# nv-tlabs/LION

Hardware: NVIDIA H100
Metric: shapes/sec (1000-step DDPM, 2048 latent pts, B=32) (higher is better)
Workload: dtype tf32 (fp32 storage/accumulate)

## Files before the change

include/lion_b200.h:

```cpp
#ifndef LION_B200_H
#define LION_B200_H
#include <stddef.h>
#ifdef __cplusplus
extern "C" {
#endif

typedef struct LionCtx LionCtx;
typedef struct LionModel LionModel;

int lion_version(void);
const char* lion_last_error(void);
int lion_ctx_create(int device, LionCtx** out);
int lion_ctx_destroy(LionCtx* ctx);
int lion_ctx_last_launches(LionCtx* ctx);
int lion_ctx_last_conv_group(LionCtx* ctx);
unsigned lion_ctx_generation(LionCtx* ctx);
int lion_ctx_timeline(LionCtx* ctx, unsigned long long* t_ns, char* names, int max_entries);
size_t lion_ctx_arena_bytes(LionCtx* ctx);
size_t lion_workspace_bytes(LionCtx* ctx);

int lion_avg_voxelize(const float* features, const int* coords, float* out, int* ind, int* cnt,
                      int B, int C, int N, int r, void* stream);
int lion_trilinear_devoxelize(const float* grid, const float* coords, float* out, int* inds, float* wgts,
                              int B, int C, int N, int r, int is_training, void* stream);
int lion_furthest_point_sampling(const float* coords, int* idx, int B, int N, int M, void* stream);
int lion_gather(const float* features, const int* idx, float* out, int B, int C, int N, int M, void* stream);
int lion_ball_query(const float* centers, const float* points, int* out, int B, int N, int M, float radius, int K,
                    void* stream);
int lion_grouping(const float* features, const int* idx, float* out, int B, int C, int N, int M, int U, void* stream);
int lion_three_nn_interpolate(const float* points, const float* centers, const float* centers_features, float* out,
                              int* idx, float* wgt, int B, int C, int N, int M, void* stream);
int lion_voxel_coords(const float* coords, float* norm_coords, int* vox, int B, int N, int r, int normalize, float eps,
                      void* stream);

int lion_avg_voxelize_backward(const float* grad_y , const int* ind , const int* cnt ,
                               float* grad_x , int B, int C, int N, int r, void* stream);
int lion_trilinear_devoxelize_backward(const float* grad_y , const int* inds , const float* wgts ,
                                       float* grad_x , int B, int C, int N, int r, void* stream);
int lion_grouping_backward(const float* grad_y , const int* idx , float* grad_x , int B, int C,
                           int N, int M, int U, void* stream);
int lion_three_nn_interpolate_backward(const float* grad_y , const int* idx , const float* wgt ,
                                       float* grad_x , int B, int C, int N, int M, void* stream);
int lion_gather_backward(const float* grad_y , const int* idx , float* grad_x , int B, int C, int N,
                         int M, void* stream);

enum { LION_KIND_UNET = 1, LION_KIND_PVCONV = 2, LION_KIND_SA = 3, LION_KIND_FP = 4, LION_KIND_ATTN = 5,
       LION_KIND_SHARED_MLP = 6, LION_KIND_GLOBAL_PRIOR = 7, LION_KIND_ADAGN = 8, LION_KIND_CONV3D = 9,
       LION_KIND_STYLE_ENC = 10 };
int lion_model_create(LionCtx* ctx, int kind, const int* desc, int ndesc, const float* const* params, int nparams,
                      LionModel** out);
int lion_model_destroy(LionModel* m);
int lion_model_refresh(LionModel* m);

int lion_unet_forward(LionModel* m, const float* x, const float* t, const float* style, const float* clip, float* out,
                      int B, int N, void* stream);
int lion_unet_cache_style(LionModel* m, const float* style, const float* clip, int B, void* stream);
int lion_style_encoder_forward(LionModel* m, const float* x, float* out, int B, int N, void* stream);
int lion_pvconv_fwd(LionModel* m, const float* features, const float* coords, const float* style, float* out,
                    int B, int N, void* stream);
int lion_sa_module_fwd(LionModel* m, const float* features, const float* coords, const float* style,
                       float* out_features, float* out_coords, int B, int N, void* stream);
int lion_fp_module_fwd(LionModel* m, const float* points_coords, const float* centers_coords,
                       const float* centers_features, const float* points_features, const float* style, float* out,
                       int B, int N, int M, void* stream);
int lion_linear_attention_fwd(LionModel* m, const float* x, float* out, int B, int N, void* stream);
int lion_shared_mlp_fwd(LionModel* m, const float* x, const float* style, float* out, int B, int R, void* stream);
int lion_adagn_fwd(LionModel* m, const float* x, const float* style, float* out, int B, int R, void* stream);
int lion_se3d_fwd(LionCtx* ctx, const float* w1, const float* w2, const float* x, float* out, int B, int C, int V, void* stream);
// ... 59 lines not shown
```

lion_b200/_lib.py:

```python
import ctypes as C
import os
import threading

import torch

_HERE = os.path.dirname(os.path.abspath(__file__))
LIB_PATH = os.path.join(_HERE, "csrc", "liblion_b200.so")


class LionError(RuntimeError):
    pass


_lib = None
_lock = threading.Lock()
c_f = C.c_void_p


def _proto(lib):
    i, f, sz, vp = C.c_int, C.c_float, C.c_size_t, C.c_void_p
    P = lambda *a: list(a)
    sig = {
        "lion_version": ([], i),
        "lion_last_error": ([], C.c_char_p),
        "lion_ctx_create": (P(i, C.POINTER(vp)), i),
        "lion_ctx_destroy": (P(vp), i),
        "lion_ctx_last_launches": (P(vp), i),
        "lion_ctx_last_conv_group": (P(vp), i),
        "lion_ctx_arena_bytes": (P(vp), sz),
        "lion_ctx_generation": (P(vp), C.c_uint),
        "lion_ctx_timeline": (P(vp, vp, vp, i), i),
        "lion_avg_voxelize": (P(vp, vp, vp, vp, vp, i, i, i, i, vp), i),
        "lion_trilinear_devoxelize": (P(vp, vp, vp, vp, vp, i, i, i, i, i, vp), i),
        "lion_furthest_point_sampling": (P(vp, vp, i, i, i, vp), i),
        "lion_gather": (P(vp, vp, vp, i, i, i, i, vp), i),
        "lion_ball_query": (P(vp, vp, vp, i, i, i, f, i, vp), i),
        "lion_grouping": (P(vp, vp, vp, i, i, i, i, i, vp), i),
        "lion_three_nn_interpolate": (P(vp, vp, vp, vp, vp, vp, i, i, i, i, vp), i),
        "lion_voxel_coords": (P(vp, vp, vp, i, i, i, i, f, vp), i),
        "lion_avg_voxelize_backward": (P(vp, vp, vp, vp, i, i, i, i, vp), i),
        "lion_trilinear_devoxelize_backward": (P(vp, vp, vp, vp, i, i, i, i, vp), i),
        "lion_grouping_backward": (P(vp, vp, vp, i, i, i, i, i, vp), i),
        "lion_three_nn_interpolate_backward": (P(vp, vp, vp, vp, i, i, i, i, vp), i),
        "lion_gather_backward": (P(vp, vp, vp, i, i, i, i, vp), i),
        "lion_model_create": (P(vp, i, C.POINTER(i), i, C.POINTER(vp), i, C.POINTER(vp)), i),
        "lion_model_destroy": (P(vp), i),
        "lion_model_refresh": (P(vp), i),
        "lion_unet_forward": (P(vp, vp, vp, vp, vp, vp, i, i, vp), i),
        "lion_unet_cache_style": (P(vp, vp, vp, i, vp), i),
        "lion_style_encoder_forward": (P(vp, vp, vp, i, i, vp), i),
        "lion_pvconv_fwd": (P(vp, vp, vp, vp, vp, i, i, vp), i),
        "lion_sa_module_fwd": (P(vp, vp, vp, vp, vp, vp, i, i, vp), i),
        "lion_fp_module_fwd": (P(vp, vp, vp, vp, vp, vp, vp, i, i, i, vp), i),
        "lion_linear_attention_fwd": (P(vp, vp, vp, i, i, vp), i),
        "lion_shared_mlp_fwd": (P(vp, vp, vp, vp, i, i, vp), i),
        "lion_global_prior_forward": (P(vp, vp, vp, vp, vp, i, vp), i),
        "lion_adagn_fwd": (P(vp, vp, vp, vp, i, i, vp), i),
        "lion_se3d_fwd": (P(vp, vp, vp, vp, vp, i, i, i, vp), i),
        "lion_swish_fwd": (P(vp, vp, sz, vp), i),
        "lion_ddpm_update": (P(vp, vp, vp, vp, vp, vp, f, sz, vp, i, vp), i),
        "lion_ddpm_set_step": (P(vp, vp, i, i, vp), i),
        "lion_ddpm_next_step": (P(vp, vp, i, vp), i),
        "lion_ddpm_fetch_noise": (P(vp, vp, vp, sz, vp), i),
        "lion_conv3d_gn_fwd": (P(vp, vp, vp, vp, vp, i, vp), i),
        "lion_pvconv_conv1_probe": (P(vp, vp, vp, i, vp, vp, vp, C.POINTER(i), i, i, vp), i),
        "lion_sa_mlp_probe": (P(vp, vp, vp, vp, i, vp, vp, vp, vp, vp, vp, C.POINTER(i), i, i, vp), i),
        "lion_pvconv_probe": (P(vp, vp, vp, vp, vp, vp, vp, vp, vp, vp, vp, vp, C.POINTER(i), i, i, vp), i),
        "lion_attention_probe": (P(vp, vp, vp, vp, vp, i, i, vp), i),
        "lion_global_prior_step": (P(vp, vp, vp, vp, vp, i, vp), i),
        "lion_workspace_bytes": (P(vp), sz),
        "lion_ddim_update": (P(vp, vp, vp, vp, vp, vp, sz, vp, vp), i),
        "lion_ddim_set_step": (P(vp, vp, vp, i, i, i, vp), i),
        "lion_ddim_next_step": (P(vp, vp, vp, i, i, vp), i),
        "lion_scheduler_step": (P(vp, vp, vp, vp, vp, vp, sz, vp), i),
        "lion_chamfer_forward": (P(vp, vp, vp, vp, vp, vp, i, i, i, vp), i),
        "lion_chamfer_pairwise": (P(vp, vp, vp, i, i, i, i, vp), i),
        "lion_chamfer_backward": (P(vp, vp, vp, vp, vp, vp, vp, vp, i, i, i, vp), i),
        "lion_emd_approx": (P(vp, vp, vp, i, i, i, vp), i),
        "lion_emd_approx_saved": (P(vp, vp, vp, vp, i, i, i, vp), i),
        "lion_emd_backward": (P(vp, vp, vp, vp, vp, vp, i, i, i, vp), i),
        "lion_emd_pairwise": (P(vp, vp, vp, i, i, i, i, vp), i),
# ... 162 lines not shown
```

lion_b200/csrc/common.cuh:

```cuda
#pragma once
#include <cuda_runtime.h>
#include <cstdint>
#include <cstdio>
#include <cstdarg>
#include <cstring>
#include <string>
#include <vector>
#include <mutex>

namespace lion {

enum : int { LION_OK = 0, LION_ERR_CUDA = -1, LION_ERR_ARG = -2, LION_ERR_OOM = -3, LION_ERR_STATE = -4 };

void set_error(const char* fmt, ...);
const char* get_error();

#define LION_CHECK_CUDA(expr)                                                          \
  do {                                                                                 \
    cudaError_t _e = (expr);                                                           \
    if (_e != cudaSuccess) {                                                           \
      lion::set_error("%s:%d: %s -> %s", __FILE__, __LINE__, #expr, cudaGetErrorString(_e)); \
      return lion::LION_ERR_CUDA;                                                      \
    }                                                                                  \
  } while (0)

#define LION_REQUIRE(cond, ...)                                                        \
  do {                                                                                 \
    if (!(cond)) {                                                                     \
      lion::set_error(__VA_ARGS__);                                                    \
      return lion::LION_ERR_ARG;                                                       \
    }                                                                                  \
  } while (0)

#define LION_TRY(expr)                                                                 \
  do {                                                                                 \
    int _r = (expr);                                                                   \
    if (_r != 0) return _r;                                                            \
  } while (0)

constexpr int LION_MAX_STAMPS = 256;
struct Ctx {
  int device = 0;
  int num_sms = 132;
  int l2_bytes = 50 << 20;
  cudaStream_t stream = nullptr;
  cudaStream_t aux = nullptr;
  char* base = nullptr;
  char* zgrid = nullptr;
  size_t zgrid_cap = 0, zgrid_need = 0;
  size_t cap = 0;
  size_t off = 0;
  size_t peak = 0;
  unsigned generation = 0;
  std::mutex* mu = nullptr;
  bool dry = false;
  int launches = 0;
  int conv_smem_cap = 0;
  int conv_group_blocks = 0;
  unsigned long long* d_stamps = nullptr;
  int n_stamps = 0;
  char stamp_names[LION_MAX_STAMPS][24];

  void reset() { off = 0; peak = 0; launches = 0; zgrid_need = 0; n_stamps = 0; }
  void* alloc(size_t bytes) {
    size_t a = (off + 255) & ~size_t(255);
    off = a + bytes;
    if (off > peak) peak = off;
    if (dry) return (void*)(uintptr_t)(0x1000 + a);
    return base + a;
  }
  template <typename T> T* alloc_n(size_t n) { return (T*)alloc(n * sizeof(T)); }
  size_t mark() const { return off; }
  void release(size_t m) { off = m; }
};

int ctx_reserve(Ctx* c, size_t bytes);

#define LION_LAUNCH_ON(ctx, stream, kernel, grid, block, smem, ...)                    \
  do {                                                                                 \
    if (!(ctx)->dry) {                                                                 \
      kernel<<<(grid), (block), (smem), (stream)>>>(__VA_ARGS__);                      \
      (ctx)->launches++;                                                               \
    }                                                                                  \
  } while (0)
#define LION_LAUNCH(ctx, kernel, grid, block, smem, ...) LION_LAUNCH_ON(ctx, (ctx)->stream, kernel, grid, block, smem, __VA_ARGS__)

static __global__ void k_stamp(unsigned long long* p) {
  unsigned long long t;
  asm volatile("mov.u64 %0, %%globaltimer;" : "=l"(t));
  *p = t;
}
inline void stamp(Ctx* c, cudaStream_t s, const char* name, int idx = -1) {
  if (!c->d_stamps || c->dry || c->n_stamps >= LION_MAX_STAMPS) return;
  const char* pre = s == c->aux ? "aux:" : "";
  if (idx >= 0) snprintf(c->stamp_names[c->n_stamps], 24, "%s%s%d", pre, name, idx);
  else snprintf(c->stamp_names[c->n_stamps], 24, "%s%s", pre, name);
  k_stamp<<<1, 1, 0, s>>>(c->d_stamps + c->n_stamps);
  c->n_stamps++;
}

inline int memset_async(Ctx* c, void* p, int v, size_t bytes, cudaStream_t s) {
  if (c->dry || bytes == 0) return 0;
  LION_CHECK_CUDA(cudaMemsetAsync(p, v, bytes, s));
  return 0;
}
inline int memset_async(Ctx* c, void* p, int v, size_t bytes) { return memset_async(c, p, v, bytes, c->stream); }
inline int memcpy_d2d(Ctx* c, void* d, const void* s, size_t bytes) {
  if (c->dry || bytes == 0) return 0;
  LION_CHECK_CUDA(cudaMemcpyAsync(d, s, bytes, cudaMemcpyDeviceToDevice, c->stream));
  return 0;
}
// ... 62 lines not shown
```

lion_b200/csrc/conv_tc.cu:

```cuda
#include <algorithm>

#include "common.cuh"
#include "model.cuh"
#include "wgmma.cuh"

namespace lion {
namespace tc {

using namespace sm90;

constexpr int CONSUMER_WARPS = 8;
constexpr int THREADS = 32 * CONSUMER_WARPS + 32;
__host__ __device__ constexpr int conv_threads(int BPW) { return BPW == 2 ? 32 * CONSUMER_WARPS + 128 : THREADS; }
constexpr int PRODUCER_REGS = 96, CONSUMER_REGS = 200;
constexpr int MAX_A_STAGES = 16;
constexpr int MAX_B_STAGES = 4;
constexpr int OCC_SMEM = 1024;
__host__ __device__ constexpr int tiles_per_item(int NT) { return NT <= 32 ? 4 : (NT <= 64 ? 2 : 1); }
constexpr int SMEM_BIAS = 128 * 4, SMEM_BARS = 64 * 8 + 128;
__host__ __device__ constexpr int smem_stat(int NT) { return CONSUMER_WARPS * 2 * NT * 4; }
__host__ __device__ constexpr int smem_pool(int NT, int TPG) { return TPG == 1 ? CONSUMER_WARPS * 2 * NT * 4 : 0; }
__host__ __device__ constexpr int smem_fixed(int NT, int TPG) {
  return SMEM_BIAS + smem_stat(NT) + smem_pool(NT, TPG) + SMEM_BARS + OCC_SMEM;
}

struct Params {
  const float4* in; const float* w; const float* bias; float4* out; double* ssum; double* ssq;
  int Gin, Gout_store, cout_pad;
  int rows;
  int p_begin, p_end;
  int ntile;
  int ntg, tpg;
  int tg_off[3];
  int tap_off[9];
  int r, rp, nzb, npl, nblk, ib;
  int halo;
  int KG, nchunk;
  int NT;
  int G;
  int B;
  int a_stage_bytes, b_stage_bytes, stage_rows;
  int a_stages;
  int b_stages;
  const unsigned char* occ;
  int occ_stride;
  float* pool_mm;
  int sched;
};

__host__ __device__ __forceinline__ int block_row(int k, int rp, int nzb, int npl) {
  const int x = k / npl, rem = k - x * npl, yb = rem / nzb, zb = rem - yb * nzb;
  return ((x + 1) * rp + 1 + 8 * yb) * rp + 1 + 8 * zb;
}

template <int KG, int TPG, int NT, int NB = 1>
__device__ __forceinline__ void issue_stage(float (*d)[NT / 2], const uint32_t* a_addr, uint32_t b_addr, uint32_t a_pitch,
                                            uint32_t a_sbo, const int* tap_off) {
  const uint64_t b0 = make_desc(b_addr, NT * 16, 128);
  uint64_t a0[NB];
#pragma unroll
  for (int k = 0; k < NB; ++k) a0[k] = make_desc(a_addr[k], a_pitch, a_sbo);
#pragma unroll
  for (int t = 0; t < TPG; ++t) {
    const uint64_t toff = (uint64_t)(int64_t)(TPG == 1 ? 0 : tap_off[t]);
#pragma unroll
    for (int ks = 0; ks < KG / 2; ++ks)
#pragma unroll
      for (int k = 0; k < NB; ++k)
        wgmma_tf32<NT>(d[k], a0[k] + toff + (uint64_t)((ks * 2 * a_pitch) >> 4), b0 + (uint64_t)(((t * KG + ks * 2) * NT * 16) >> 4), 1);
  }
}


struct Items {
  long long u, u_end; int ntile_total, B, G;
  int mode, m, q, n_p, n_q, c_i, i, big, k;
  __device__ __forceinline__ bool next(int& nt, long long& v0, int& ntile) {
    const long long per_nt = (long long)B * ntile_total;
    if (mode) {
      while (u >= u_end) {
        if (k >= m) return false;
        const int a0 = q * k / m, a1 = q * (k + 1) / m, b0 = (q + 1) * k / m, b1 = (q + 1) * (k + 1) / m;
        u = (long long)n_q * a0 + (long long)n_p * b0 + (long long)(i - c_i) * (a1 - a0) + (long long)c_i * (b1 - b0);
        u_end = u + (big ? b1 - b0 : a1 - a0);
        ++k;
      }
      nt = (int)(u / per_nt);
      v0 = u - (long long)nt * per_nt;
      const long long lim = (long long)(nt + 1) * per_nt;
      const long long e = u_end < lim ? u_end : lim;
      ntile = (int)(e - u);
      u = e;
      return true;
    }
    if (u >= u_end) return false;
    nt = (int)(u / per_nt);
// ... 1 lines not shown
    long long run = per_nt - v0;
    if (u_end - u < run) run = u_end - u;
    const long long k2 = (run + G - 1) / G;
    ntile = (int)((run + k2 - 1) / k2);
    u += ntile;
    return true;
  }
};
__device__ __forceinline__ Items make_items(long long U, int ntile_total, int B, int G, int sched) {
  const long long u_begin = U * blockIdx.x / gridDim.x, u_end = U * (blockIdx.x + 1) / gridDim.x;
  Items it{u_begin, u_end, ntile_total, B, G, 0, 0, 0, 0, 0, 0, 0, 0, 0};
  if (sched) {
    const int grid = (int)gridDim.x, q = (int)(U / grid), n_p = (int)(U - (long long)q * grid);
    const int tmax = q + (n_p ? 1 : 0);
    it.mode = 1; it.u = 0; it.u_end = 0;
    it.m = (tmax + G - 1) / G; it.q = q; it.n_p = n_p; it.n_q = grid - n_p;
    it.i = (int)blockIdx.x; it.c_i = (int)(u_begin - (long long)q * blockIdx.x);
    it.big = (int)(u_end - u_begin) > q; it.k = 0;
  }
  return it;
}

__device__ __forceinline__ void halo_mask(int p_lo, int rp, bool& ok_lo, bool& ok_hi) {
  const int p_hi = p_lo + 8;
  const int z0 = p_lo % rp, y0 = (p_lo / rp) % rp, z1 = p_hi % rp, y1 = (p_hi / rp) % rp;
  ok_lo = ok_lo && z0 >= 1 && z0 <= rp - 2 && y0 >= 1 && y0 <= rp - 2;
  ok_hi = ok_hi && z1 >= 1 && z1 <= rp - 2 && y1 >= 1 && y1 <= rp - 2;
}
template <int NT>
__device__ __forceinline__ void stat_add(float* s_stat, int cw, int lane, int col, float x0, float x1, float x2, float x3) {
  const float s0 = red8<0>(x0 + x2), s1 = red8<0>(x1 + x3);
  const float q0 = red8<0>(fmaf(x0, x0, x2 * x2)), q1 = red8<0>(fmaf(x1, x1, x3 * x3));
  if (lane < 4) {
    float* st = s_stat + (cw * 2) * NT + col;
    st[0] += s0; st[1] += s1; st[NT] += q0; st[NT + 1] += q1;
  }
}
template <int NT>
__device__ __forceinline__ void stat_flush(const Params& P, float* s_stat, int et, int b, int n0) {
  asm volatile("bar.sync 1, 256;" ::: "memory");
  if (et < NT) {
    float s = 0.f, qq = 0.f;
#pragma unroll
    for (int w = 0; w < CONSUMER_WARPS; ++w) {
      s += s_stat[(w * 2 + 0) * NT + et]; qq += s_stat[(w * 2 + 1) * NT + et];
      s_stat[(w * 2 + 0) * NT + et] = 0.0f; s_stat[(w * 2 + 1) * NT + et] = 0.0f;
    }
    atomicAdd(P.ssum + (size_t)b * P.cout_pad + n0 + et, (double)s);
    atomicAdd(P.ssq + (size_t)b * P.cout_pad + n0 + et, (double)qq);
  }
  asm volatile("bar.sync 1, 256;" ::: "memory");
}

template <int KG, int TPG, int NT, bool BLK, int BPW = 1>
__global__ void __launch_bounds__(conv_threads(BPW), 1) k_conv_tc(Params P) {
  constexpr int GT = BLK ? BPW : tiles_per_item(NT);
  constexpr int NTHR = conv_threads(BPW);
  constexpr bool SETREG = NTHR > THREADS;
  constexpr int NACC = NT / 2;
  extern __shared__ __align__(128) uint8_t smem[];
  uint8_t* sA = smem;
  const int A_STAGES = P.a_stages;
  uint8_t* sB = sA + (size_t)A_STAGES * P.a_stage_bytes;
  const int B_STAGES = P.b_stages;
  float* s_bias = (float*)(sB + (size_t)B_STAGES * P.b_stage_bytes);
  float* s_stat = s_bias + 128;
  float* s_pool = s_stat + CONSUMER_WARPS * 2 * NT;
  uint64_t* bars = (uint64_t*)((uint8_t*)s_stat + smem_stat(NT) + smem_pool(NT, TPG));
  volatile uint32_t* s_skip = (volatile uint32_t*)(bars + 64);
  uint8_t* s_occ = (uint8_t*)(bars + 64) + 128;
  const int tid = threadIdx.x, warp = tid >> 5, lane = tid & 31;

  const uint32_t bar_full_a = smem_u32(bars), bar_empty_a = smem_u32(bars + MAX_A_STAGES);
  const uint32_t bar_full_b = smem_u32(bars + 2 * MAX_A_STAGES), bar_empty_b = smem_u32(bars + 2 * MAX_A_STAGES + MAX_B_STAGES);

  if (P.Gin % KG != 0)
    for (int i = tid; i < A_STAGES * P.a_stage_bytes / 16; i += NTHR) ((float4*)sA)[i] = make_float4(0.f, 0.f, 0.f, 0.f);
  for (int i = tid; i < CONSUMER_WARPS * 2 * NT; i += NTHR) s_stat[i] = 0.0f;
  if (tid == 0) {
    for (int i = 0; i < A_STAGES; ++i) { mbar_init(bar_full_a + 8 * i, 1); mbar_init(bar_empty_a + 8 * i, CONSUMER_WARPS); }
    for (int i = 0; i < B_STAGES; ++i) { mbar_init(bar_full_b + 8 * i, 1); mbar_init(bar_empty_b + 8 * i, CONSUMER_WARPS); }
    asm volatile("fence.mbarrier_init.release.cluster;" ::: "memory");
  }
  asm volatile("fence.proxy.async.shared::cta;" ::: "memory");
  __syncthreads();

  const int ntile_total = P.ntile;
  const int n_nt = P.cout_pad / P.NT;
  const long long U = (long long)n_nt * P.B * ntile_total;
  const Items items0 = make_items(U, ntile_total, P.B, P.G, P.sched);

  if (warp >= CONSUMER_WARPS) {
    if constexpr (SETREG) {
      regs_dec<PRODUCER_REGS>();
      if (warp > CONSUMER_WARPS) return;
    }
    uint32_t sa = 0, pa = 0, sb = 0, pb = 0;
    const uint32_t bytes = (uint32_t)P.stage_rows * 16u;
    const uint32_t sA_addr = smem_u32(sA), sB_addr = smem_u32(sB);
    Items items = items0;
    int nt, ntile;
    long long v0;
    int occ_shape = -1;
    while (items.next(nt, v0, ntile)) {
      const float* wsrc = P.w + (size_t)nt * P.nchunk * P.ntg * (P.b_stage_bytes / 4);
      int my_b = 0, my_t = 0;
      if (lane < ntile) { const int vl = (int)v0 + lane; my_b = vl / ntile_total; my_t = vl - my_b * ntile_total; }
      for (int cc = 0; cc < P.nchunk; ++cc) {
        const int kg_real = min(KG, P.Gin - cc * KG);
        const size_t grp_lane = (size_t)(cc * KG + (lane < kg_real ? lane : 0));
        for (int tg = 0; tg < P.ntg; ++tg) {
          const bool may_skip = P.occ && !(cc == P.nchunk - 1 && tg == P.ntg - 1);
          mbar_wait<SETREG>(bar_empty_b + 8 * sb, pb ^ 1);
          if (lane == 0) {
            mbar_expect_tx(bar_full_b + 8 * sb, P.b_stage_bytes);
            bulk_g2s(sB_addr + sb * (uint32_t)P.b_stage_bytes, wsrc + (size_t)(cc * P.ntg + tg) * (P.b_stage_bytes / 4),
                     P.b_stage_bytes, bar_full_b + 8 * sb);
          }
          if (++sb == B_STAGES) { sb = 0; pb ^= 1; }
          for (int j = 0; j < ntile; ++j) {
            const int bj = __shfl_sync(0xffffffffu, my_b, j), tj = __shfl_sync(0xffffffffu, my_t, j);
            long long row0;
            uint32_t cnt = (uint32_t)P.stage_rows;
            if (!BLK) {
              row0 = (long long)P.p_begin + (long long)tj * 128 - P.halo + P.tg_off[tg];
            } else {
              row0 = (long long)block_row(tj * P.ib, P.rp, P.nzb, P.npl) - P.rp - 1 + P.tg_off[tg];
              if (row0 + cnt > (long long)P.rows) cnt = (uint32_t)(P.rows - row0);
            }
            const float4* in_lane = P.in + ((size_t)bj * P.Gin + grp_lane) * P.rows;
            mbar_wait<SETREG>(bar_empty_a + 8 * sa, pa ^ 1);
            bool empty = false;
            if (may_skip) {
              const unsigned char* occ_b = P.occ + (size_t)bj * P.occ_stride;
              if (P.occ_stride <= OCC_SMEM) {
                if (occ_shape != bj) {
                  __syncwarp();
                  for (int k = lane; k < P.occ_stride; k += 32) s_occ[k] = __ldg(occ_b + k);
                  __syncwarp();
                  occ_shape = bj;
                }
                occ_b = s_occ;
              }
              long long lo = row0 < 0 ? 0 : row0, hi = row0 + cnt - 1;
              if (hi > P.rows - 1) hi = P.rows - 1;
              unsigned any = 0;
              for (int k = (int)(lo >> 6); k <= (int)(hi >> 6); ++k) any |= occ_b[k];
              empty = (any == 0);
            }
            const uint32_t full = bar_full_a + 8 * sa;
            if (lane == 0) {
              s_skip[sa] = empty ? 1u : 0u;
              if (empty) asm volatile("mbarrier.arrive.release.cta.shared::cta.b64 _, [%0];" ::"r"(full) : "memory");
              else mbar_expect_tx(full, cnt * 16u * kg_real);
            }
            __syncwarp();
            if (!empty && lane < kg_real)
              bulk_g2s(sA_addr + sa * (uint32_t)P.a_stage_bytes + lane * bytes, in_lane + row0, cnt * 16u, full);
            if (++sa == (uint32_t)A_STAGES) { sa = 0; pa ^= 1; }
          }
        }
      }
    }
  } else {
    if constexpr (SETREG) regs_inc<CONSUMER_REGS>();
    const int cw = warp, wg = cw >> 2, wq = cw & 3;
    const int et = tid;
    const uint32_t a_pitch = (uint32_t)P.stage_rows * 16u;
    const uint32_t a_sbo = BLK ? (uint32_t)P.rp * 16u : 128u;
    const uint32_t a_ring = smem_u32(sA) + (BLK ? 0u : (uint32_t)(P.halo + 64 * wg) * 16u);
    const uint32_t b_ring = smem_u32(sB);
    const int r_lo = 64 * wg + 16 * wq + (lane >> 2);
    const int c_lo = 2 * (lane & 3);
    const bool odd = (lane & 1) != 0;
    float acc[GT][NACC];
    uint32_t sa = 0, pa = 0, sb = 0, pb = 0;
    Items items = items0;
    int nt, ntile;
    long long v0;
    auto release = [&](int& s, uint32_t bar0) {
      if (s >= 0) { if (lane == 0) mbar_arrive(bar0 + 8 * s); s = -1; }
    };
    while (items.next(nt, v0, ntile)) {
#pragma unroll
      for (int j = 0; j < GT; ++j)
#pragma unroll
        for (int i = 0; i < NACC; ++i) acc[j][i] = 0.0f;
      int g_f = 0, nbw = 0;
      uint32_t boff[GT];
      if (BLK) {
        const int g_b = (int)(v0 / ntile_total);
        g_f = (int)(v0 - (long long)g_b * ntile_total) * P.ib;
        const int nb = min(P.ib, P.nblk - g_f);
        nbw = (nb - wg + 1) / 2;
        const int s_f = block_row(g_f, P.rp, P.nzb, P.npl);
#pragma unroll
        for (int j = 0; j < GT; ++j) {
          const int k = 2 * j + wg < nb ? g_f + 2 * j + wg : g_f;
          boff[j] = (uint32_t)(block_row(k, P.rp, P.nzb, P.npl) - s_f + P.rp + 1) * 16u;
        }
      }
      int pend_a = -1, pend_b = -1;
      for (int cc = 0; cc < P.nchunk; ++cc) {
        for (int tg = 0; tg < P.ntg; ++tg) {
          mbar_wait<SETREG>(bar_full_b + 8 * sb, pb);
          const uint32_t b_addr = b_ring + sb * (uint32_t)P.b_stage_bytes;
#pragma unroll
          for (int j = 0; j < (BLK ? 1 : GT); ++j) {
            if (j < ntile) {
              mbar_wait<SETREG>(bar_full_a + 8 * sa, pa);
              const uint32_t a_addr = a_ring + sa * (uint32_t)P.a_stage_bytes;
              if (!s_skip[sa]) {
                wg_fence();
                if (!BLK) {
                  issue_stage<KG, TPG, NT>(&acc[j], &a_addr, b_addr, a_pitch, a_sbo, P.tap_off);
                } else {
                  uint32_t a_blk[GT];
#pragma unroll
                  for (int k = 0; k < GT; ++k) a_blk[k] = a_addr + boff[k];
                  issue_stage<KG, TPG, NT, GT>(acc, a_blk, b_addr, a_pitch, a_sbo, P.tap_off);
                }
                wg_commit();
                wg_wait<1>();
                release(pend_a, bar_empty_a);
                release(pend_b, bar_empty_b);
                pend_a = (int)sa;
              } else {
                int s = (int)sa;
                release(s, bar_empty_a);
              }
              if (++sa == (uint32_t)A_STAGES) { sa = 0; pa ^= 1; }
            }
          }
          if (pend_b >= 0) {
            wg_wait<0>();
            release(pend_a, bar_empty_a);
            release(pend_b, bar_empty_b);
          }
          if (pend_a >= 0) pend_b = (int)sb;
          else { int s = (int)sb; release(s, bar_empty_b); }
          if (++sb == B_STAGES) { sb = 0; pb ^= 1; }
        }
      }
      wg_wait<0>();
      release(pend_a, bar_empty_a);
      release(pend_b, bar_empty_b);
#pragma unroll
      for (int j = 0; j < GT; ++j) fence_regs<NACC>(acc[j]);

      const int n0 = nt * NT;
      asm volatile("bar.sync 1, 256;" ::: "memory");
      if (et < NT) s_bias[et] = P.bias ? P.bias[n0 + et] : 0.0f;
      asm volatile("bar.sync 1, 256;" ::: "memory");
      int b = (int)(v0 / ntile_total);
#pragma unroll
      for (int j = 0; j < GT; ++j) {
        if (j < (BLK ? nbw : ntile)) {
          int tj = 0, p_lo, p_hi;
          bool ok_lo, ok_hi;
          bool in_lo, in_hi;
          if (!BLK) {
            const long long vj = v0 + j;
            const int bj = (int)(vj / ntile_total);
            tj = (int)(vj - (long long)bj * ntile_total);
            if (bj != b) { if (P.ssum) stat_flush<NT>(P, s_stat, et, b, n0); b = bj; }
            p_lo = P.p_begin + tj * 128 + r_lo; p_hi = p_lo + 8;
            in_lo = p_lo < P.p_end; in_hi = p_hi < P.p_end;
            ok_lo = in_lo; ok_hi = in_hi;
            if (TPG != 1) halo_mask(p_lo, P.rp, ok_lo, ok_hi);
          } else {
            const int k = g_f + 2 * j + wg, x = k / P.npl, rem = k - x * P.npl, yb = rem / P.nzb, zb = rem - yb * P.nzb;
            const int y = 1 + 8 * yb + 2 * wq, z = 1 + 8 * zb + (lane >> 2);
            p_lo = ((x + 1) * P.rp + y) * P.rp + z; p_hi = p_lo + P.rp;
            ok_lo = y <= P.r && z <= P.r; ok_hi = y + 1 <= P.r && z <= P.r;
            in_lo = ok_lo; in_hi = ok_hi;
          }
#pragma unroll
          for (int i = 0; i < NT / 8; ++i) {
            const int col = 8 * i + c_lo;
            const float x0 = ok_lo ? acc[j][4 * i + 0] + s_bias[col] : 0.0f, x1 = ok_lo ? acc[j][4 * i + 1] + s_bias[col + 1] : 0.0f;
            const float x2 = ok_hi ? acc[j][4 * i + 2] + s_bias[col] : 0.0f, x3 = ok_hi ? acc[j][4 * i + 3] + s_bias[col + 1] : 0.0f;
            if (P.ssum) stat_add<NT>(s_stat, cw, lane, col, x0, x1, x2, x3);
            if (TPG == 1 && P.pool_mm) {
              const float mn0 = red8<1>(fminf(x0, x2)), mn1 = red8<1>(fminf(x1, x3));
              const float mx0 = red8<2>(fmaxf(x0, x2)), mx1 = red8<2>(fmaxf(x1, x3));
              if (lane < 4) {
                float* sp = s_pool + (cw * 2) * NT + col;
                sp[0] = mn0; sp[1] = mn1; sp[NT] = mx0; sp[NT + 1] = mx1;
              }
            } else {
              const float y0 = __shfl_xor_sync(0xffffffffu, odd ? x0 : x2, 1);
              const float y1 = __shfl_xor_sync(0xffffffffu, odd ? x1 : x3, 1);
              const int g = (n0 + 8 * i + (lane & 2) * 2) >> 2;
              if (g < P.Gout_store) {
// ... 84 lines not shown
  int cc = r % nchunk; r /= nchunk;
  int nt = (int)r;
  int tap = tg * tpg + t;
  int ci = (cc * KG + kg) * 4 + jj;
  float v = 0.0f;
  if (ci < cin_pad) v = wt[((size_t)tap * cin_pad + ci) * cout_pad + nt * NT + n];
  uint32_t u;
  asm("cvt.rna.tf32.f32 %0, %1;" : "=r"(u) : "f"(v));
  w[i] = __uint_as_float(u);
}

}

int conv_tc_prepare(Model* m, ConvW& w) {
  w.tc = ConvTcW();
  if (!(w.ntaps == 27 || w.ntaps == 1)) return 0;
  if (w.cout_pad < 32 || w.cout_pad % 32) return 0;
  ConvTcW t;
  t.NT = w.cout_pad < 128 ? w.cout_pad : 128;
  if (w.cout_pad % t.NT) return 0;
  t.ntg = w.ntaps == 27 ? 3 : 1;
  t.tpg = w.ntaps == 27 ? 9 : 1;
  const int G = w.cin_pad / 4;
  t.KG = (w.ntaps == 27 && t.NT > 64) ? 4 : 8;
  if (G < t.KG) t.KG = (G <= 2) ? 2 : ((G <= 4) ? 4 : 8);
  t.nchunk = (G + t.KG - 1) / t.KG;
  const size_t total = (size_t)(w.cout_pad / t.NT) * t.nchunk * t.ntg * t.tpg * t.KG * t.NT * 4;
  LION_TRY(m->dmalloc(&t.w, total));
  w.tc = t;
  m->repack.push_back([t, wt = w.wt, ntaps = w.ntaps, cin_pad = w.cin_pad, cout_pad = w.cout_pad, total] {
    tc::k_pack_tc<<<(unsigned)cdivz(total, 256), 256>>>(wt, t.w, ntaps, cin_pad, cout_pad, t.NT, t.nchunk, t.ntg, t.tpg, t.KG);
  });
  return 0;
}

bool conv_tc_usable(const ConvW& w, const ConvGeom& geo) {
  if (!w.tc.w) return false;
  if (geo.ntaps != w.ntaps) return false;
  return true;
}

int conv_tc_run(Ctx* c, const ConvW& w, const float4* in, int Gin, float4* out, int Gout_store, double* ssum, double* ssq,
                const ConvGeom& geo, int B, float* pool_mm) {
  tc::Params P{};
  if (pool_mm && (w.ntaps != 1 || geo.p_begin != 0 || geo.p_end != geo.rows || geo.rows % 128)) {
    set_error("conv_tc: the pooled epilogue needs a 1x1 convolution over a multiple of 128 rows"); return LION_ERR_ARG;
  }
  P.pool_mm = pool_mm;
  const int NT = w.tc.NT, KG = w.tc.KG, tpg = w.tc.tpg;
  P.in = in; P.w = w.tc.w; P.bias = w.bias; P.out = out; P.ssum = ssum; P.ssq = ssq;
  P.Gin = Gin; P.Gout_store = Gout_store; P.cout_pad = w.cout_pad;
  P.rows = geo.rows; P.p_begin = geo.p_begin; P.p_end = geo.p_end;
  P.ntg = w.tc.ntg; P.tpg = tpg; P.KG = KG; P.nchunk = w.tc.nchunk; P.NT = NT;
  P.b_stage_bytes = tpg * KG * NT * 16;
  P.B = B;
  P.occ = geo.occ; P.occ_stride = geo.occ_stride;
  const size_t fixed = tc::smem_fixed(NT, tpg);
  const bool blk = w.ntaps == 27 && NT == 128;
  const int ntile_rows = cdiv(geo.p_end - geo.p_begin, 128);
  int ntile;
  P.halo = 0;
  if (w.ntaps == 27) {
    const int rp = geo.rp, r = rp - 2;
    for (int dx = 0; dx < 3; ++dx) P.tg_off[dx] = (dx - 1) * rp * rp;
    for (int dy = 0; dy < 3; ++dy) for (int dz = 0; dz < 3; ++dz) P.tap_off[dy * 3 + dz] = (dy - 1) * rp + (dz - 1);
    P.r = r; P.rp = rp;
  } else {
    P.tg_off[0] = 0; P.tap_off[0] = 0;
  }
  const int n_tiles_n = w.cout_pad / NT;
  if (blk) {
    const int rp = P.rp, r = P.r;
    P.nzb = cdiv(r, 8); P.npl = P.nzb * P.nzb; P.nblk = r * P.npl;
    auto window_rows = [&](int ib) {
      int wrows = 0;
      for (int f = 0; f < P.nblk; f += ib) {
        const int l = std::min(f + ib, P.nblk) - 1;
        wrows = std::max(wrows, tc::block_row(l, rp, P.nzb, P.npl) - tc::block_row(f, rp, P.nzb, P.npl) + 9 * rp + 10);
      }
      return wrows;
    };
    const long long a_room2 = 227LL * 1024 - (long long)fixed - 2LL * P.b_stage_bytes;
    const bool four = (long long)n_tiles_n * B * cdiv(P.nblk, 4) >= c->num_sms && a_room2 / (KG * window_rows(4) * 16) >= 3;
    P.ib = four ? 4 : 2;
    P.stage_rows = window_rows(P.ib);
    ntile = cdiv(P.nblk, P.ib);
    P.G = 1;
  } else {
    if (w.ntaps == 27) P.halo = P.rp + 1;
    P.stage_rows = 128 + 2 * P.halo;
    ntile = ntile_rows;
    P.G = tc::tiles_per_item(NT);
  }
  P.ntile = ntile;
  P.a_stage_bytes = KG * P.stage_rows * 16;
  int b_stages = 2;
  if (blk) {
    const long long limit = (c->conv_smem_cap > 0 ? c->conv_smem_cap : 227LL * 1024) - (long long)fixed;
    while (b_stages < tc::MAX_B_STAGES &&
           (limit - (long long)(b_stages + 1) * P.b_stage_bytes) / P.a_stage_bytes >= std::max(4, b_stages + 1))
      ++b_stages;
  }
  P.b_stages = b_stages;
  const long long a_room = 227LL * 1024 - (long long)fixed - (long long)b_stages * P.b_stage_bytes;
  const double in_bytes = (double)B * Gin * geo.rows * 16.0;
  P.sched = w.ntaps == 27 && in_bytes > 1.6 * c->l2_bytes ? 1 : 0;
  int a_stages = (int)(a_room / P.a_stage_bytes);
  if (c->conv_smem_cap > 0 && a_stages >= 5) {
    int capped = (int)(((long long)c->conv_smem_cap - (long long)fixed - (long long)b_stages * P.b_stage_bytes) / P.a_stage_bytes);
    if (capped >= 4 && capped < a_stages) a_stages = capped;
  }
  if (a_stages > tc::MAX_A_STAGES) a_stages = tc::MAX_A_STAGES;
  if (a_stages < 2) { set_error("conv_tc: shared memory cannot hold the operand pipeline (N=%d, KG=%d)", NT, KG); return LION_ERR_ARG; }
  P.a_stages = a_stages;
  if (!blk && P.occ && a_stages < 2 * P.G) P.occ = nullptr;
  size_t smem = (size_t)a_stages * P.a_stage_bytes + (size_t)b_stages * P.b_stage_bytes + fixed;
  if (smem > 227 * 1024) { set_error("conv_tc: %zu bytes of shared memory needed", smem); return LION_ERR_ARG; }
  auto grid_for = [&](int nt_per_shape) {
    long long n_units = (long long)nt_per_shape * n_tiles_n * B;
    long long per_cta = (n_units + c->num_sms - 1) / c->num_sms;
    return (int)((n_units + per_cta - 1) / per_cta);
  };
  const int grid = grid_for(ntile);
  tc::Params S = P;
  if (blk && ssum) {
    P.ssum = nullptr; P.ssq = nullptr;
    S.ntile = ntile_rows; S.G = tc::tiles_per_item(NT);
  }
  auto stats = [&]() -> int {
    if (!(blk && ssum)) return 0;
    LION_LAUNCH(c, tc::k_conv_stats<128>, grid_for(ntile_rows), 256, 0, S);
    return check_launch(c, "conv_tc stats");
  };
  const int bpw = blk ? P.ib / 2 : 1;
  c->conv_group_blocks = blk ? P.ib : 0;
#define CONV_TC_CASE(kg, tpg_, nt_, blk_, bpw_)                                                           \
  if (KG == kg && tpg == tpg_ && NT == nt_ && blk == blk_ && bpw == bpw_) {                               \
    static DevOnce attr_once;                                                                             \
    if (attr_once.need()) {                                                                               \
      LION_CHECK_CUDA(cudaFuncSetAttribute(tc::k_conv_tc<kg, tpg_, nt_, blk_, bpw_>, cudaFuncAttributeMaxDynamicSharedMemorySize, 227 * 1024)); \
    }                                                                                                     \
    LION_LAUNCH(c, (tc::k_conv_tc<kg, tpg_, nt_, blk_, bpw_>), grid, tc::conv_threads(bpw_), smem, P);    \
    LION_TRY(check_launch(c, "conv_tc"));                                                                 \
    return stats();                                                                                       \
  }
#define CONV_TC_NT(kg, tpg_) CONV_TC_CASE(kg, tpg_, 32, false, 1) CONV_TC_CASE(kg, tpg_, 64, false, 1) CONV_TC_CASE(kg, tpg_, 96, false, 1)
  CONV_TC_NT(2, 1) CONV_TC_NT(4, 1) CONV_TC_NT(8, 1) CONV_TC_NT(2, 9) CONV_TC_NT(4, 9) CONV_TC_NT(8, 9)
  CONV_TC_CASE(2, 1, 128, false, 1) CONV_TC_CASE(4, 1, 128, false, 1) CONV_TC_CASE(8, 1, 128, false, 1)
  CONV_TC_CASE(2, 9, 128, true, 1) CONV_TC_CASE(4, 9, 128, true, 1) CONV_TC_CASE(2, 9, 128, true, 2) CONV_TC_CASE(4, 9, 128, true, 2)
#undef CONV_TC_NT
#undef CONV_TC_CASE
  set_error("conv_tc: no kernel for N=%d, KG=%d, %d taps", NT, KG, tpg);
  return LION_ERR_ARG;
}

}
```

lion_b200/csrc/net.cu:

```cuda
#include <algorithm>
#include <deque>
#include <memory>
#include <cstdlib>
#include <cmath>
#include "common.cuh"
#include "packed_kernels.cuh"
#include "model.cuh"
#include "../../include/lion_b200.h"

namespace lion {

static thread_local char g_err[1024] = "";
void set_error(const char* fmt, ...) {
  va_list ap;
  va_start(ap, fmt);
  vsnprintf(g_err, sizeof(g_err), fmt, ap);
  va_end(ap);
}
const char* get_error() { return g_err; }

int ctx_reserve(Ctx* c, size_t bytes) {
  if (bytes <= c->cap) return 0;
  cudaStreamCaptureStatus st = cudaStreamCaptureStatusNone;
  cudaStreamIsCapturing(c->stream, &st);
// ... 991 lines not shown
    Fwd f{c, m, B};
    int rc = body(f);
    if (rc) { c->dry = false; return rc; }
    if (pass == 0) {
      LION_TRY(ctx_reserve(c, c->peak));
      LION_TRY(ctx_reserve_zgrid(c, c->zgrid_need));
    }
  }
  return 0;
}

}

using namespace lion;

struct LionCtx { Ctx c; std::mutex mu; };
struct LionModel { Model m; };

extern "C" int lion_version(void) { return 100; }
extern "C" const char* lion_last_error(void) { return get_error(); }

extern "C" int lion_ctx_create(int device, LionCtx** out) {
  LION_REQUIRE(out, "lion_ctx_create: null out");
  LION_CHECK_CUDA(cudaSetDevice(device));
  LionCtx* h = new LionCtx();
  h->c.device = device;
  h->c.mu = &h->mu;
  cudaDeviceProp prop;
  LION_CHECK_CUDA(cudaGetDeviceProperties(&prop, device));
  h->c.num_sms = prop.multiProcessorCount;
  h->c.l2_bytes = prop.l2CacheSize;
  LION_CHECK_CUDA(cudaStreamCreateWithFlags(&h->c.aux, cudaStreamNonBlocking));
  { const char* e = getenv("LION_TIMELINE");
    if (e && atoi(e) != 0) LION_CHECK_CUDA(cudaMalloc(&h->c.d_stamps, LION_MAX_STAMPS * sizeof(unsigned long long))); }
  if (prop.major != 9 || prop.minor != 0) {
    set_error("lion_b200 is built for sm_90a only; device %d is sm_%d%d", device, prop.major, prop.minor);
    delete h;
    return LION_ERR_STATE;
  }
  *out = h;
  return 0;
}
extern "C" int lion_ctx_destroy(LionCtx* h) {
  if (!h) return 0;
  if (h->c.base) cudaFree(h->c.base);
  if (h->c.zgrid) cudaFree(h->c.zgrid);
  if (h->c.aux) cudaStreamDestroy(h->c.aux);
  if (h->c.d_stamps) cudaFree(h->c.d_stamps);
  delete h;
  return 0;
}
extern "C" int lion_ctx_last_launches(LionCtx* h) { return h ? h->c.launches : 0; }
extern "C" int lion_ctx_last_conv_group(LionCtx* h) { return h ? h->c.conv_group_blocks : 0; }
extern "C" unsigned lion_ctx_generation(LionCtx* h) { return h ? h->c.generation : 0; }
extern "C" int lion_ctx_timeline(LionCtx* h, unsigned long long* t_ns, char* names, int max_entries) {
  LION_REQUIRE(h && t_ns && names && max_entries >= 0, "lion_ctx_timeline: null argument");
  if (!h->c.d_stamps) { set_error("lion_ctx_timeline: the context was created without LION_TIMELINE=1"); return LION_ERR_STATE; }
  int n = h->c.n_stamps < max_entries ? h->c.n_stamps : max_entries;
  LION_CHECK_CUDA(cudaSetDevice(h->c.device));
  LION_CHECK_CUDA(cudaDeviceSynchronize());
  LION_CHECK_CUDA(cudaMemcpy(t_ns, h->c.d_stamps, (size_t)n * sizeof(unsigned long long), cudaMemcpyDeviceToHost));
  for (int i = 0; i < n; ++i) memcpy(names + (size_t)i * 24, h->c.stamp_names[i], 24);
  return n;
}
extern "C" size_t lion_ctx_arena_bytes(LionCtx* h) { return h ? h->c.cap : 0; }
extern "C" size_t lion_workspace_bytes(LionCtx* h) { return h ? h->c.cap + h->c.zgrid_cap : 0; }

extern "C" int lion_model_create(LionCtx* ctx, int kind, const int* desc, int ndesc, const float* const* params,
                                 int nparams, LionModel** out) {
  LION_REQUIRE(ctx && out && (desc || ndesc == 0) && (params || nparams == 0), "lion_model_create: null argument");
  LION_CHECK_CUDA(cudaSetDevice(ctx->c.device));
  std::unique_ptr<LionModel> h(new LionModel());
  Model* m = &h->m;
  m->ctx = &ctx->c; m->kind = kind;
  m->desc.assign(desc, desc + ndesc);
  m->params.assign(params, params + nparams);
  for (int i = 0; i < nparams; ++i) LION_REQUIRE(params[i], "lion_model_create: parameter %d is null", i);
  Cursor cur{m->params.data(), nparams};
  const std::vector<int>& d = m->desc;
  auto need = [&](int n) { return (int)d.size() >= n; };
  switch (kind) {
    case LION_KIND_UNET: LION_TRY(build_unet(m, cur)); break;
    case LION_KIND_PVCONV: {
      LION_REQUIRE(need(5), "pvconv descriptor: [cin, cout, r, attn, style_dim]");
      m->S = d[4] > 0 ? d[4] : 4;
      m->block.reset(new Block()); m->block->kind = kind;
      LION_TRY(make_pvconv(m, m->block->pv, cur, d[0], d[1], d[2], d[3] != 0, d[4] == 0));
      break;
    }
    case LION_KIND_SA: {
      LION_REQUIRE(need(6) && need(6 + d[5]), "sa descriptor: [cfeat, m, radius_bits, k, style_dim, n, outs...]");
      m->S = d[4] > 0 ? d[4] : 4;
      m->block.reset(new Block()); m->block->kind = kind;
      LION_TRY(make_sa(m, m->block->sa, cur, d[0], d[1], bits_to_float(d[2]), d[3], std::vector<int>(d.begin() + 6, d.begin() + 6 + d[5]), d[4] == 0));
      break;
    }
    case LION_KIND_FP: {
      LION_REQUIRE(need(4) && need(4 + d[3]), "fp descriptor: [cc, cp, style_dim, n, outs...]");
      m->S = d[2];
      m->block.reset(new Block()); m->block->kind = kind;
      LION_TRY(make_fp(m, m->block->fp, cur, d[0], d[1], std::vector<int>(d.begin() + 4, d.begin() + 4 + d[3])));
      break;
    }
    case LION_KIND_ATTN: {
      LION_REQUIRE(need(2), "attention descriptor: [C, heads]");
      LION_REQUIRE(d[0] % 4 == 0, "attention: C must be a multiple of 4");
// ... 464 lines not shown
```

Measured before the change: 2.931.

## Split 27-tap conv weight slabs into 3-tap stages to deepen activation ring

For the blocked tensor-core 3D conv path, each 9-tap weight slab is now streamed as three 3-tap stages through a deeper weight ring. The shared memory this frees goes to more activation stages. The consumer issues partial-tap MMAs per stage and reuses the same A stage across parts, and a host heuristic picks split mode only when it yields more A stages than the whole-slab layout. The cost is more barrier waits and smaller MMA batches per stage, plus extra template instantiations and a toggle to force whole slabs.

Result: faster. 3.053, median of 6 (+4.2%).

```diff
diff --git a/include/lion_b200.h b/include/lion_b200.h
--- a/include/lion_b200.h
+++ b/include/lion_b200.h
@@ -14,6 +14,8 @@
 int lion_ctx_destroy(LionCtx* ctx);
 int lion_ctx_last_launches(LionCtx* ctx);
 int lion_ctx_last_conv_group(LionCtx* ctx);
+int lion_ctx_last_conv_stage_taps(LionCtx* ctx);
+int lion_ctx_set_conv_whole_slabs(LionCtx* ctx, int on);
 unsigned lion_ctx_generation(LionCtx* ctx);
 int lion_ctx_timeline(LionCtx* ctx, unsigned long long* t_ns, char* names, int max_entries);
 size_t lion_ctx_arena_bytes(LionCtx* ctx);
diff --git a/lion_b200/_lib.py b/lion_b200/_lib.py
--- a/lion_b200/_lib.py
+++ b/lion_b200/_lib.py
@@ -27,6 +27,8 @@
         "lion_ctx_destroy": (P(vp), i),
         "lion_ctx_last_launches": (P(vp), i),
         "lion_ctx_last_conv_group": (P(vp), i),
+        "lion_ctx_last_conv_stage_taps": (P(vp), i),
+        "lion_ctx_set_conv_whole_slabs": (P(vp, i), i),
         "lion_ctx_arena_bytes": (P(vp), sz),
         "lion_ctx_generation": (P(vp), C.c_uint),
         "lion_ctx_timeline": (P(vp, vp, vp, i), i),
diff --git a/lion_b200/csrc/common.cuh b/lion_b200/csrc/common.cuh
--- a/lion_b200/csrc/common.cuh
+++ b/lion_b200/csrc/common.cuh
@@ -57,6 +57,8 @@
   int launches = 0;
   int conv_smem_cap = 0;
   int conv_group_blocks = 0;
+  int conv_stage_taps = 0;
+  bool conv_whole_slabs = false;
   unsigned long long* d_stamps = nullptr;
   int n_stamps = 0;
   char stamp_names[LION_MAX_STAMPS][24];
diff --git a/lion_b200/csrc/conv_tc.cu b/lion_b200/csrc/conv_tc.cu
--- a/lion_b200/csrc/conv_tc.cu
+++ b/lion_b200/csrc/conv_tc.cu
@@ -42,6 +42,7 @@
   int a_stage_bytes, b_stage_bytes, stage_rows;
   int a_stages;
   int b_stages;
+  int tps;
   const unsigned char* occ;
   int occ_stride;
   float* pool_mm;
@@ -149,12 +150,13 @@
   asm volatile("bar.sync 1, 256;" ::: "memory");
 }
 
-template <int KG, int TPG, int NT, bool BLK, int BPW = 1>
+template <int KG, int TPG, int NT, bool BLK, int BPW = 1, int TPS = TPG>
 __global__ void __launch_bounds__(conv_threads(BPW), 1) k_conv_tc(Params P) {
   constexpr int GT = BLK ? BPW : tiles_per_item(NT);
   constexpr int NTHR = conv_threads(BPW);
   constexpr bool SETREG = NTHR > THREADS;
   constexpr int NACC = NT / 2;
+  constexpr int NPARTS = TPG / TPS;
   extern __shared__ __align__(128) uint8_t smem[];
   uint8_t* sA = smem;
   const int A_STAGES = P.a_stages;
@@ -199,8 +201,17 @@
     int nt, ntile;
     long long v0;
     int occ_shape = -1;
+    const int slab_floats = P.tpg * KG * NT * 4;
+    auto copy_weights = [&](const float* src) {
+      mbar_wait<SETREG>(bar_empty_b + 8 * sb, pb ^ 1);
+      if (lane == 0) {
+        mbar_expect_tx(bar_full_b + 8 * sb, P.b_stage_bytes);
+        bulk_g2s(sB_addr + sb * (uint32_t)P.b_stage_bytes, src, P.b_stage_bytes, bar_full_b + 8 * sb);
+      }
+      if (++sb == B_STAGES) { sb = 0; pb ^= 1; }
+    };
     while (items.next(nt, v0, ntile)) {
-      const float* wsrc = P.w + (size_t)nt * P.nchunk * P.ntg * (P.b_stage_bytes / 4);
+      const float* wsrc = P.w + (size_t)nt * P.nchunk * P.ntg * slab_floats;
       int my_b = 0, my_t = 0;
       if (lane < ntile) { const int vl = (int)v0 + lane; my_b = vl / ntile_total; my_t = vl - my_b * ntile_total; }
       for (int cc = 0; cc < P.nchunk; ++cc) {
@@ -208,13 +219,8 @@
         const size_t grp_lane = (size_t)(cc * KG + (lane < kg_real ? lane : 0));
         for (int tg = 0; tg < P.ntg; ++tg) {
           const bool may_skip = P.occ && !(cc == P.nchunk - 1 && tg == P.ntg - 1);
-          mbar_wait<SETREG>(bar_empty_b + 8 * sb, pb ^ 1);
-          if (lane == 0) {
-            mbar_expect_tx(bar_full_b + 8 * sb, P.b_stage_bytes);
-            bulk_g2s(sB_addr + sb * (uint32_t)P.b_stage_bytes, wsrc + (size_t)(cc * P.ntg + tg) * (P.b_stage_bytes / 4),
-                     P.b_stage_bytes, bar_full_b + 8 * sb);
-          }
-          if (++sb == B_STAGES) { sb = 0; pb ^= 1; }
+          const float* slab = wsrc + (size_t)(cc * P.ntg + tg) * slab_floats;
+          copy_weights(slab);
           for (int j = 0; j < ntile; ++j) {
             const int bj = __shfl_sync(0xffffffffu, my_b, j), tj = __shfl_sync(0xffffffffu, my_t, j);
             long long row0;
@@ -256,6 +262,7 @@
               bulk_g2s(sA_addr + sa * (uint32_t)P.a_stage_bytes + lane * bytes, in_lane + row0, cnt * 16u, full);
             if (++sa == (uint32_t)A_STAGES) { sa = 0; pa ^= 1; }
           }
+          for (int s = 1; s < NPARTS; ++s) copy_weights(slab + (size_t)s * (P.b_stage_bytes / 4));
         }
       }
     }
@@ -298,45 +305,55 @@
         }
       }
       int pend_a = -1, pend_b = -1;
+      bool skip[BLK ? 1 : GT];
       for (int cc = 0; cc < P.nchunk; ++cc) {
         for (int tg = 0; tg < P.ntg; ++tg) {
-          mbar_wait<SETREG>(bar_full_b + 8 * sb, pb);
-          const uint32_t b_addr = b_ring + sb * (uint32_t)P.b_stage_bytes;
-#pragma unroll
-          for (int j = 0; j < (BLK ? 1 : GT); ++j) {
-            if (j < ntile) {
-              mbar_wait<SETREG>(bar_full_a + 8 * sa, pa);
-              const uint32_t a_addr = a_ring + sa * (uint32_t)P.a_stage_bytes;
-              if (!s_skip[sa]) {
-                wg_fence();
-                if (!BLK) {
-                  issue_stage<KG, TPG, NT>(&acc[j], &a_addr, b_addr, a_pitch, a_sbo, P.tap_off);
-                } else {
-                  uint32_t a_blk[GT];
-#pragma unroll
-                  for (int k = 0; k < GT; ++k) a_blk[k] = a_addr + boff[k];
-                  issue_stage<KG, TPG, NT, GT>(acc, a_blk, b_addr, a_pitch, a_sbo, P.tap_off);
+          const uint32_t sa0 = sa, pa0 = pa;
+#pragma unroll
+          for (int s = 0; s < NPARTS; ++s) {
+            mbar_wait<SETREG>(bar_full_b + 8 * sb, pb);
+            const uint32_t b_addr = b_ring + sb * (uint32_t)P.b_stage_bytes;
+            const int* toff = P.tap_off + s * TPS;
+            bool issued = false;
+            sa = sa0; pa = pa0;
+#pragma unroll
+            for (int j = 0; j < (BLK ? 1 : GT); ++j) {
+              if (j < ntile) {
+                if (s == 0) {
+                  mbar_wait<SETREG>(bar_full_a + 8 * sa, pa);
+                  skip[j] = s_skip[sa] != 0;
+                  if (skip[j]) { int st = (int)sa; release(st, bar_empty_a); }
                 }
-                wg_commit();
-                wg_wait<1>();
-                release(pend_a, bar_empty_a);
-                release(pend_b, bar_empty_b);
-                pend_a = (int)sa;
-              } else {
-                int s = (int)sa;
-                release(s, bar_empty_a);
+                if (!skip[j]) {
+                  const uint32_t a_addr = a_ring + sa * (uint32_t)P.a_stage_bytes;
+                  wg_fence();
+                  if (!BLK) {
+                    issue_stage<KG, TPS, NT>(&acc[j], &a_addr, b_addr, a_pitch, a_sbo, toff);
+                  } else {
+                    uint32_t a_blk[GT];
+#pragma unroll
+                    for (int k = 0; k < GT; ++k) a_blk[k] = a_addr + boff[k];
+                    issue_stage<KG, TPS, NT, GT>(acc, a_blk, b_addr, a_pitch, a_sbo, toff);
+                  }
+                  wg_commit();
+                  wg_wait<1>();
+                  release(pend_a, bar_empty_a);
+                  release(pend_b, bar_empty_b);
+                  if (s == NPARTS - 1) pend_a = (int)sa;
+                  issued = true;
+                }
+                if (++sa == (uint32_t)A_STAGES) { sa = 0; pa ^= 1; }
               }
-              if (++sa == (uint32_t)A_STAGES) { sa = 0; pa ^= 1; }
             }
+            if (pend_b >= 0) {
+              wg_wait<0>();
+              release(pend_a, bar_empty_a);
+              release(pend_b, bar_empty_b);
+            }
+            if (issued) pend_b = (int)sb;
+            else { int st = (int)sb; release(st, bar_empty_b); }
+            if (++sb == B_STAGES) { sb = 0; pb ^= 1; }
           }
-          if (pend_b >= 0) {
-            wg_wait<0>();
-            release(pend_a, bar_empty_a);
-            release(pend_b, bar_empty_b);
-          }
-          if (pend_a >= 0) pend_b = (int)sb;
-          else { int s = (int)sb; release(s, bar_empty_b); }
-          if (++sb == B_STAGES) { sb = 0; pb ^= 1; }
         }
       }
       wg_wait<0>();
@@ -527,7 +544,7 @@
   P.Gin = Gin; P.Gout_store = Gout_store; P.cout_pad = w.cout_pad;
   P.rows = geo.rows; P.p_begin = geo.p_begin; P.p_end = geo.p_end;
   P.ntg = w.tc.ntg; P.tpg = tpg; P.KG = KG; P.nchunk = w.tc.nchunk; P.NT = NT;
-  P.b_stage_bytes = tpg * KG * NT * 16;
+  const int slab_bytes = tpg * KG * NT * 16;
   P.B = B;
   P.occ = geo.occ; P.occ_stride = geo.occ_stride;
   const size_t fixed = tc::smem_fixed(NT, tpg);
@@ -555,7 +572,7 @@
       }
       return wrows;
     };
-    const long long a_room2 = 227LL * 1024 - (long long)fixed - 2LL * P.b_stage_bytes;
+    const long long a_room2 = 227LL * 1024 - (long long)fixed - 2LL * slab_bytes;
     const bool four = (long long)n_tiles_n * B * cdiv(P.nblk, 4) >= c->num_sms && a_room2 / (KG * window_rows(4) * 16) >= 3;
     P.ib = four ? 4 : 2;
     P.stage_rows = window_rows(P.ib);
@@ -569,25 +586,37 @@
   }
   P.ntile = ntile;
   P.a_stage_bytes = KG * P.stage_rows * 16;
-  int b_stages = 2;
-  if (blk) {
-    const long long limit = (c->conv_smem_cap > 0 ? c->conv_smem_cap : 227LL * 1024) - (long long)fixed;
-    while (b_stages < tc::MAX_B_STAGES &&
-           (limit - (long long)(b_stages + 1) * P.b_stage_bytes) / P.a_stage_bytes >= std::max(4, b_stages + 1))
-      ++b_stages;
-  }
-  P.b_stages = b_stages;
-  const long long a_room = 227LL * 1024 - (long long)fixed - (long long)b_stages * P.b_stage_bytes;
   const double in_bytes = (double)B * Gin * geo.rows * 16.0;
   P.sched = w.ntaps == 27 && in_bytes > 1.6 * c->l2_bytes ? 1 : 0;
-  int a_stages = (int)(a_room / P.a_stage_bytes);
-  if (c->conv_smem_cap > 0 && a_stages >= 5) {
-    int capped = (int)(((long long)c->conv_smem_cap - (long long)fixed - (long long)b_stages * P.b_stage_bytes) / P.a_stage_bytes);
-    if (capped >= 4 && capped < a_stages) a_stages = capped;
-  }
-  if (a_stages > tc::MAX_A_STAGES) a_stages = tc::MAX_A_STAGES;
-  if (a_stages < 2) { set_error("conv_tc: shared memory cannot hold the operand pipeline (N=%d, KG=%d)", NT, KG); return LION_ERR_ARG; }
+  auto ring = [&](int tps, int& b_stages) -> int {
+    const long long stage = (long long)slab_bytes / tpg * tps;
+    b_stages = tps == tpg ? 2 : tc::MAX_B_STAGES;
+    if (blk && tps == tpg) {
+      const long long limit = (c->conv_smem_cap > 0 ? c->conv_smem_cap : 227LL * 1024) - (long long)fixed;
+      while (b_stages < tc::MAX_B_STAGES && (limit - (b_stages + 1) * stage) / P.a_stage_bytes >= std::max(4, b_stages + 1))
+        ++b_stages;
+    }
+    int a_stages = (int)((227LL * 1024 - (long long)fixed - b_stages * stage) / P.a_stage_bytes);
+    if (c->conv_smem_cap > 0 && a_stages >= 5) {
+      const int capped = (int)(((long long)c->conv_smem_cap - (long long)fixed - b_stages * stage) / P.a_stage_bytes);
+      if (capped >= 4 && capped < a_stages) a_stages = capped;
+    }
+    a_stages = std::min(a_stages, tc::MAX_A_STAGES);
+    return a_stages >= 2 ? a_stages : 0;
+  };
+  int b_whole = 0, b_parts = 0;
+  const int a_whole = ring(tpg, b_whole);
+  const int a_parts = blk && !c->conv_whole_slabs ? ring(3, b_parts) : 0;
+  const bool parts = a_parts > a_whole && a_parts >= P.G + 1;
+  if (!parts && !a_whole) {
+    set_error("conv_tc: shared memory cannot hold the operand pipeline (N=%d, KG=%d)", NT, KG); return LION_ERR_ARG;
+  }
+  P.tps = parts ? 3 : tpg;
+  P.b_stage_bytes = slab_bytes / tpg * P.tps;
+  P.b_stages = parts ? b_parts : b_whole;
+  const int a_stages = parts ? a_parts : a_whole;
   P.a_stages = a_stages;
+  const int b_stages = P.b_stages;
   if (!blk && P.occ && a_stages < 2 * P.G) P.occ = nullptr;
   size_t smem = (size_t)a_stages * P.a_stage_bytes + (size_t)b_stages * P.b_stage_bytes + fixed;
   if (smem > 227 * 1024) { set_error("conv_tc: %zu bytes of shared memory needed", smem); return LION_ERR_ARG; }
@@ -609,23 +638,26 @@
   };
   const int bpw = blk ? P.ib / 2 : 1;
   c->conv_group_blocks = blk ? P.ib : 0;
-#define CONV_TC_CASE(kg, tpg_, nt_, blk_, bpw_)                                                           \
-  if (KG == kg && tpg == tpg_ && NT == nt_ && blk == blk_ && bpw == bpw_) {                               \
+  c->conv_stage_taps = P.tps;
+#define CONV_TC_CASE(kg, tpg_, nt_, blk_, bpw_, tps_)                                                     \
+  if (KG == kg && tpg == tpg_ && NT == nt_ && blk == blk_ && bpw == bpw_ && P.tps == tps_) {              \
     static DevOnce attr_once;                                                                             \
     if (attr_once.need()) {                                                                               \
-      LION_CHECK_CUDA(cudaFuncSetAttribute(tc::k_conv_tc<kg, tpg_, nt_, blk_, bpw_>, cudaFuncAttributeMaxDynamicSharedMemorySize, 227 * 1024)); \
+      LION_CHECK_CUDA(cudaFuncSetAttribute(tc::k_conv_tc<kg, tpg_, nt_, blk_, bpw_, tps_>, cudaFuncAttributeMaxDynamicSharedMemorySize, 227 * 1024)); \
     }                                                                                                     \
-    LION_LAUNCH(c, (tc::k_conv_tc<kg, tpg_, nt_, blk_, bpw_>), grid, tc::conv_threads(bpw_), smem, P);    \
+    LION_LAUNCH(c, (tc::k_conv_tc<kg, tpg_, nt_, blk_, bpw_, tps_>), grid, tc::conv_threads(bpw_), smem, P); \
     LION_TRY(check_launch(c, "conv_tc"));                                                                 \
     return stats();                                                                                       \
   }
-#define CONV_TC_NT(kg, tpg_) CONV_TC_CASE(kg, tpg_, 32, false, 1) CONV_TC_CASE(kg, tpg_, 64, false, 1) CONV_TC_CASE(kg, tpg_, 96, false, 1)
+#define CONV_TC_NT(kg, tpg_) CONV_TC_CASE(kg, tpg_, 32, false, 1, tpg_) CONV_TC_CASE(kg, tpg_, 64, false, 1, tpg_) CONV_TC_CASE(kg, tpg_, 96, false, 1, tpg_)
+#define CONV_TC_BLK(kg, bpw_) CONV_TC_CASE(kg, 9, 128, true, bpw_, 9) CONV_TC_CASE(kg, 9, 128, true, bpw_, 3)
   CONV_TC_NT(2, 1) CONV_TC_NT(4, 1) CONV_TC_NT(8, 1) CONV_TC_NT(2, 9) CONV_TC_NT(4, 9) CONV_TC_NT(8, 9)
-  CONV_TC_CASE(2, 1, 128, false, 1) CONV_TC_CASE(4, 1, 128, false, 1) CONV_TC_CASE(8, 1, 128, false, 1)
-  CONV_TC_CASE(2, 9, 128, true, 1) CONV_TC_CASE(4, 9, 128, true, 1) CONV_TC_CASE(2, 9, 128, true, 2) CONV_TC_CASE(4, 9, 128, true, 2)
+  CONV_TC_CASE(2, 1, 128, false, 1, 1) CONV_TC_CASE(4, 1, 128, false, 1, 1) CONV_TC_CASE(8, 1, 128, false, 1, 1)
+  CONV_TC_BLK(2, 1) CONV_TC_BLK(4, 1) CONV_TC_BLK(2, 2) CONV_TC_BLK(4, 2)
 #undef CONV_TC_NT
+#undef CONV_TC_BLK
 #undef CONV_TC_CASE
-  set_error("conv_tc: no kernel for N=%d, KG=%d, %d taps", NT, KG, tpg);
+  set_error("conv_tc: no kernel for N=%d, KG=%d, %d taps, %d per weight stage", NT, KG, tpg, P.tps);
   return LION_ERR_ARG;
 }
 
diff --git a/lion_b200/csrc/net.cu b/lion_b200/csrc/net.cu
--- a/lion_b200/csrc/net.cu
+++ b/lion_b200/csrc/net.cu
@@ -1067,6 +1067,12 @@
 }
 extern "C" int lion_ctx_last_launches(LionCtx* h) { return h ? h->c.launches : 0; }
 extern "C" int lion_ctx_last_conv_group(LionCtx* h) { return h ? h->c.conv_group_blocks : 0; }
+extern "C" int lion_ctx_last_conv_stage_taps(LionCtx* h) { return h ? h->c.conv_stage_taps : 0; }
+extern "C" int lion_ctx_set_conv_whole_slabs(LionCtx* h, int on) {
+  LION_REQUIRE(h, "lion_ctx_set_conv_whole_slabs: null context");
+  h->c.conv_whole_slabs = on != 0;
+  return 0;
+}
 extern "C" unsigned lion_ctx_generation(LionCtx* h) { return h ? h->c.generation : 0; }
 extern "C" int lion_ctx_timeline(LionCtx* h, unsigned long long* t_ns, char* names, int max_entries) {
   LION_REQUIRE(h && t_ns && names && max_entries >= 0, "lion_ctx_timeline: null argument");
```
